# Tuxliri/RL_rocket

Hardware: AMD Instinct MI355X
Metric: env-steps/sec (6DOF, N=65536 per GPU) (higher is better)
Workload: dtype fp32

## Files before the change

### rl_rocket_amd/batch.py

```python
import ctypes

import numpy as np

from . import _lib
from .params import lower, make_config


def _ptr(t):
    return ctypes.c_void_p(t.data_ptr()) if t is not None else None


def _host_view(addr, shape, dtype):
    nbytes = int(np.prod(shape)) * np.dtype(dtype).itemsize
    return np.frombuffer((ctypes.c_char * nbytes).from_address(addr), dtype=dtype).reshape(shape)


class HostArray:

    def __init__(self, shape, dtype):
        self._lib = _lib.load()
        nbytes = max(1, int(np.prod(shape)) * np.dtype(dtype).itemsize)
        p = ctypes.c_void_p()
        _lib.check(self._lib.rr_host_alloc(ctypes.byref(p), nbytes), "rr_host_alloc")
        self.ptr = p
# ... 195 lines not shown
    def checkpoint(self):
        t = self.torch
        st, v0, _ = self.get_state()
        cw = t.empty((self.num_envs,), dtype=t.int32, device=self.device)
        ret = t.empty((self.num_envs,), dtype=t.float32, device=self.device)
        _lib.check(self.lib.rr_get_aux(self._h, _ptr(cw), _ptr(ret), self._stream()), "rr_get_aux")
        return {"state": st, "v0": v0, "counter": cw, "ep_return": ret}

    def restore(self, ck):
        self.set_state(ck["state"], v0=ck["v0"], elapsed=ck["counter"])
        cw, ret = ck["counter"].contiguous(), ck["ep_return"].contiguous()
        self._keep_aux = (cw, ret)
        _lib.check(self.lib.rr_set_aux(self._h, _ptr(cw), _ptr(ret), self._stream()), "rr_set_aux")

    def set_state64(self, state_soa, v0=None, elapsed=None):
        t = self.torch
        st = t.as_tensor(state_soa, device=self.device, dtype=t.float64).reshape(self.state_dim, self.num_envs)
        st = st.contiguous()
        v = None if v0 is None else t.as_tensor(v0, device=self.device, dtype=t.float32).reshape(-1).contiguous()
        el = None if elapsed is None else t.as_tensor(elapsed, device=self.device, dtype=t.int32).reshape(-1).contiguous()
        self._keep = (st, v, el)
        _lib.check(self.lib.rr_set_state64(self._h, _ptr(st), _ptr(v), _ptr(el), self._stream()), "rr_set_state64")

    def get_state64(self):
        t = self.torch
        st = t.empty((self.state_dim, self.num_envs), dtype=t.float64, device=self.device)
        v = t.empty((self.num_envs,), dtype=t.float32, device=self.device)
        el = t.empty((self.num_envs,), dtype=t.int32, device=self.device)
        _lib.check(self.lib.rr_get_state64(self._h, _ptr(st), _ptr(v), _ptr(el), self._stream()), "rr_get_state64")
        return st, v, el

    def fetch_done(self, capacity=None):
        cap = self.num_envs if capacity is None else min(int(capacity), self.num_envs)
        rows = min(cap, max(4096, len(self._fetch[0].array) if getattr(self, "_fetch", None) else 0))
        while True:
            if getattr(self, "_fetch", None) is None or len(self._fetch[0].array) < rows:
                self._free_fetch()
                ns = self.state_dim
                self._fetch = (HostArray((rows,), np.int32), HostArray((rows, ns), np.float32),
                               HostArray((rows,), np.float32), HostArray((rows,), np.int32))
            bufs = self._fetch
            c = self.lib.rr_fetch_done(self._h, min(cap, rows), *(b.ptr for b in bufs), self._stream())
            _lib.check(c, "rr_fetch_done")
            if int(c) <= rows or rows >= cap:
                break
            rows = min(cap, 1 << (int(c) - 1).bit_length())
        m = min(int(c), cap)
        return tuple(b.array[:m].copy() for b in bufs)

    def _free_fetch(self):
        for b in getattr(self, "_fetch", None) or ():
            b.free()
        self._fetch = None

    def copy_terminal(self, out=None):
        t = self.torch
        if out is None:
            out = (t.zeros((self.num_envs, self.state_dim), dtype=t.float32, device=self.device),
                   t.zeros((self.num_envs,), dtype=t.float32, device=self.device),
                   t.zeros((self.num_envs,), dtype=t.int32, device=self.device))
        tobs, ret, ln = out
        _lib.check(self.lib.rr_copy_terminal(self._h, _ptr(tobs), _ptr(ret), _ptr(ln), self._stream()),
                   "rr_copy_terminal")
        return tobs, ret, ln

    def close(self):
        if getattr(self, "_h", None) is not None and self._h.value:
            self.torch.cuda.synchronize(self.device)
            self.lib.rr_destroy(self._h)
            self._h = ctypes.c_void_p()
        self._free_fetch()

    def __del__(self):
        try:
            self.close()
        except Exception:
            pass
```

### rl_rocket_amd/build.py

```python
import os
import shutil
import subprocess
import sys

HERE = os.path.dirname(os.path.abspath(__file__))
ROOT = os.path.dirname(HERE)
SRC = os.path.join(HERE, "csrc", "rocket_hip.hip")
SRC_EXACT = os.path.join(HERE, "csrc", "rocket_exact.hip")
EXACT_FLAGS = ["-mllvm", "-amdgpu-schedule-metric-bias=100"]
SRC_COLLECT = os.path.join(HERE, "csrc", "rocket_collect.hip")
COLLECT_FLAGS = ["-mllvm", "-amdgpu-mfma-vgpr-form"]
SRC_EVAL_TRACE = os.path.join(HERE, "csrc", "eval_trace", "rocket_eval_trace.hip")
SRC_EVAL_EXACT = os.path.join(HERE, "csrc", "eval_exact", "rocket_eval_exact.hip")
EVAL_EXACT_FLAGS = EXACT_FLAGS + COLLECT_FLAGS
SRC_COLLECT_STATS = os.path.join(HERE, "csrc", "collect_stats", "rocket_collect_stats.hip")
INC_COLLECT_STATS = os.path.join(HERE, "csrc", "collect_stats", "rocket_collect_stats.inc")
SRC_PPO_OPTS = os.path.join(HERE, "csrc", "ppo_opts", "rocket_ppo_opts.hip")
SRC_BC = os.path.join(HERE, "csrc", "bc", "rocket_bc.hip")
SRC_DISCRETE = os.path.join(HERE, "csrc", "discrete", "rocket_discrete.hip")
HEADER = os.path.join(ROOT, "include", "rocket_hip.h")
OUT = os.path.join(HERE, "librocket_hip.so")
BENCH_SRC = os.path.join(ROOT, "tools", "bench_timed.hip")
BENCH_OUT = os.path.join(ROOT, "tools", "libbench_timed.so")
ARCH = os.environ.get("RR_OFFLOAD_ARCH", "gfx950")


def hipcc():
    for c in (os.environ.get("HIPCC"), shutil.which("hipcc"), "/opt/rocm/bin/hipcc"):
        if c and os.path.exists(c):
            return c
    raise RuntimeError("hipcc not found")


def command(resource_usage=False, out=OUT, defines=(), extra=(), src=SRC, compile_only=False, preload=4):
    cmd = [hipcc(), "--offload-arch=%s" % ARCH, "-O3", "-fno-slp-vectorize", "-ffp-contract=on", "-std=c++17",
           "-fPIC", "-c" if compile_only else "-shared"] + \
        (["-mllvm", "-amdgpu-kernarg-preload-count=%d" % preload] if preload else []) + \
        ["-I", os.path.join(ROOT, "include"), "-I", os.path.join(HERE, "csrc")] + list(extra) + \
        ["-D%s" % d for d in defines] + ["-o", out, src]
    if resource_usage:
        cmd.insert(1, "-Rpass-analysis=kernel-resource-usage")
    return cmd


def sources():
    csrc = os.path.join(HERE, "csrc")
    return sorted([os.path.join(csrc, f) for f in os.listdir(csrc) if os.path.isfile(os.path.join(csrc, f))]
                  + [SRC_EVAL_TRACE, SRC_EVAL_EXACT, SRC_COLLECT_STATS, INC_COLLECT_STATS, SRC_PPO_OPTS, SRC_BC, SRC_DISCRETE,
                     HEADER])


def source_hash():
    import hashlib

    h = hashlib.sha256()
    for path in sources():
        with open(path, "rb") as f:
            h.update(f.read())
    for cmd in commands():
        h.update(" ".join(cmd[1:]).replace(ROOT, "").encode())
    return h.hexdigest()[:16]


def commands(resource_usage=False, out=OUT, defines=(), extra=(), preload=4):
    o_main, o_exact, o_coll, o_trace = out + ".main.o", out + ".exact.o", out + ".collect.o", out + ".evaltrace.o"
    o_evx = out + ".evalexact.o"
    c1 = command(resource_usage, o_main, defines, extra, SRC, compile_only=True, preload=preload)
    c2 = command(resource_usage, o_exact, defines, list(extra) + EXACT_FLAGS, SRC_EXACT, compile_only=True,
                 preload=preload)
    c3 = command(resource_usage, o_coll, defines, list(extra) + COLLECT_FLAGS, SRC_COLLECT, compile_only=True,
                 preload=preload)
    c4 = command(resource_usage, o_trace, defines, list(extra) + COLLECT_FLAGS, SRC_EVAL_TRACE, compile_only=True,
                 preload=preload)
    c5 = command(resource_usage, o_evx, defines, list(extra) + EVAL_EXACT_FLAGS, SRC_EVAL_EXACT, compile_only=True,
                 preload=preload)
    objs = [o_main, o_exact, o_coll, o_trace, o_evx]
    c6 = command(resource_usage, out, defines, list(extra) + COLLECT_FLAGS + objs + [SRC_PPO_OPTS, SRC_BC, SRC_DISCRETE],
                 SRC_COLLECT_STATS,
                 preload=preload)
    return [c1, c2, c3, c4, c5, c6]


def build_lib(out=OUT, defines=(), extra=(), resource_usage=False, verbose=True, preload=4):
    cmds = commands(resource_usage, out, defines, extra, preload=preload)
    if verbose:
        for c in cmds:
            print("[rl_rocket_amd.build]", " ".join(c), flush=True)
    procs = [subprocess.Popen(c, cwd=ROOT) for c in cmds[:-1]]
    rcs = [p.wait() for p in procs]
    for c, rc in zip(cmds, rcs):
        if rc:
            raise subprocess.CalledProcessError(rc, c)
    subprocess.check_call(cmds[-1], cwd=ROOT)
    for c in cmds[:-1]:
        os.remove(c[c.index("-o") + 1])
    return out


def _llvm(tool):
    for d in (os.environ.get("ROCM_PATH", "/opt/rocm") + "/lib/llvm/bin", "/opt/rocm/llvm/bin"):
        if os.path.exists(os.path.join(d, tool)):
            return os.path.join(d, tool)
    found = shutil.which(tool)
    if not found:
        raise RuntimeError("%s not found" % tool)
    return found


def _elf_symbols(blob):
    import struct
# ... 85 lines not shown
```

### rl_rocket_amd/csrc/rocket_hip.hip

```cpp


#include <algorithm>
#include <cmath>
#include <cstdlib>
#include <cstring>
#include <new>
#include <string>
#include <vector>

#include "rocket_device.h"
#define RR_POL_PREFETCH_A 0
#include "rocket_policy.inc"
#include "rocket_rollout.inc"
#include "rocket_eval.inc"
#include "rocket_ppo.inc"

namespace {

__device__ __forceinline__ void entry_barrier()
{
    __builtin_amdgcn_fence(__ATOMIC_RELEASE, "workgroup", "local");
    __builtin_amdgcn_s_barrier();
    __builtin_amdgcn_fence(__ATOMIC_ACQUIRE, "workgroup", "local");
}

template <int MODEL, int INTEG, bool ASOA, bool HELP, int WPB, bool ROWS>
__global__ __launch_bounds__(HELP ? 2 * WPB * kWave : WPB * kWave) __attribute__((amdgpu_waves_per_eu(4))) void step_kernel(
    float* __restrict__ state, const float* __restrict__ action, uint32_t n_envs, uint32_t mode, const KParams P,
    const Bufs B, const StepIO io)
{
    constexpr int NS = Dims<MODEL>::NS, NA = Dims<MODEL>::NA, NT = Dims<MODEL>::NT, EV = Dims<MODEL>::EV;
    constexpr int OW = ROWS ? NS + 2 : NS;
    __shared__ __attribute__((aligned(16))) float lds[WPB][kWave * OW];
    constexpr int kCandRow = (NS + 1 + 3) / 4 * 4;
    __shared__ __attribute__((aligned(16))) float cand[HELP ? WPB : 1][HELP ? kWave * kCandRow : 1];
    __shared__ uint32_t cflag[WPB];
    const uint32_t lane = threadIdx.x & (kWave - 1);
    const uint32_t wv = __builtin_amdgcn_readfirstlane(threadIdx.x / kWave);
    const uint32_t n = n_envs;
    RR_STAMPS_BEGIN(4);
    RR_SUB_BEGIN(3);
    if constexpr (HELP) {
        if (wv >= (uint32_t)WPB) {
            const KParams& P = *B.kp;
            const uint32_t k = wv - WPB;
            const uint32_t base = (blockIdx.x * WPB + k) * kWave;
            const uint32_t ih = min(base + lane, n - 1);
            const uint32_t cwh = (base < n && (mode & kModeCounter)) ? at(B.counter, ih) : 0u;
// ... 142 lines not shown
    const int64_t i = (int64_t)blockIdx.x * kBlock + threadIdx.x;
    if (i >= B.n) return;
    const int64_t n = B.n;
    float s[NS], v0;
    if (mask == nullptr || mask[i]) {
        const uint32_t ep = (B.counter[i] >> P.ep_shift) + 1u;
        ResetStream key = reset_stream(B.kp->seed_w, P.id_off + i, B.counter[i]);
        sample_ic<MODEL>(P, key, s, v0);
#pragma unroll
        for (int j = 0; j < NS; ++j) B.state[(int64_t)j * n + i] = s[j];
        if (state64) {
#pragma unroll
            for (int j = 0; j < NS; ++j) state64[(int64_t)j * n + i] = (double)s[j];
        }
        B.v0[i] = v0;
        B.counter[i] = ep << P.ep_shift;
        B.ep_ret[i] = 0.0f;
    } else {
#pragma unroll
        for (int j = 0; j < NS; ++j) s[j] = B.state[(int64_t)j * n + i];
    }
    if (obs) {
#pragma unroll
        for (int j = 0; j < NS; ++j) obs[i * NS + j] = s[j] * P.inv_norm[j];
    }
}

__global__ __launch_bounds__(kBlock) void clear_elapsed_kernel(uint32_t* counter, int64_t n, uint32_t el_mask)
{
    const int64_t i = (int64_t)blockIdx.x * kBlock + threadIdx.x;
    if (i < n) counter[i] &= ~el_mask;
}

__global__ __launch_bounds__(kBlock) void gather_done_kernel(const int32_t* idx, int64_t count, int ns,
                                                             const float* term_obs, const float* term_ret,
                                                             const int32_t* term_len, const uint8_t* trunc,
                                                             float* g_obs, float* g_ret, int32_t* g_len,
                                                             uint8_t* g_trunc)
{
    const int64_t k = (int64_t)blockIdx.x * kBlock + threadIdx.x;
    if (k >= count) return;
    const int64_t i = idx[k];
    for (int j = 0; j < ns; ++j) g_obs[k * ns + j] = term_obs[i * ns + j];
    g_ret[k] = term_ret[i];
    g_len[k] = term_len[i];
    if (trunc) g_trunc[k] = trunc[i];
}

__global__ __launch_bounds__(kBlock) void copy_done_rows_kernel(const uint64_t* done_bits, int64_t n, int ns,
                                                                const float* term_obs, const float* term_ret,
                                                                const int32_t* term_len, float* d_obs, float* d_ret,
                                                                int32_t* d_len)
{
    const int64_t i = (int64_t)blockIdx.x * kBlock + threadIdx.x;
    if (i >= n || !((done_bits[i / kWave] >> (i % kWave)) & 1ull)) return;
    if (d_obs)
        for (int j = 0; j < ns; ++j) d_obs[i * ns + j] = term_obs[i * ns + j];
    if (d_ret) d_ret[i] = term_ret[i];
    if (d_len) d_len[i] = term_len[i];
}

__global__ __launch_bounds__(kBlock) void gae_kernel(int64_t T, int64_t n, const float* __restrict__ rewards,
                                                     const float* __restrict__ values,
                                                     const float* __restrict__ starts,
                                                     const float* __restrict__ last_value,
                                                     const float* __restrict__ last_done, double gamma, double lam,
                                                     float* __restrict__ adv, float* __restrict__ ret)
{
    const int64_t e = (int64_t)blockIdx.x * kBlock + threadIdx.x;
    if (e >= n) return;
    pol::gae_env(T, n, e, rewards, values, starts, last_value[e], last_done[e], gamma, lam, adv, ret);
}

__global__ __launch_bounds__(kBlock) void widen_kernel(const float* src, double* dst, int64_t count)
{
    const int64_t k = (int64_t)blockIdx.x * kBlock + threadIdx.x;
    if (k < count) dst[k] = (double)src[k];
}

__global__ __launch_bounds__(kBlock) void narrow_kernel(const double* src, float* dst, int64_t count)
{
    const int64_t k = (int64_t)blockIdx.x * kBlock + threadIdx.x;
    if (k < count) dst[k] = (float)src[k];
}

}

constexpr int kNoUnit = (int)hipErrorInvalidDeviceFunction;
extern "C" {
__attribute__((weak)) int rrx_launch_exact(const void*, const void*) { return kNoUnit; }
__attribute__((weak)) int rrx_launch_eval_exact(const void*, const void*) { return kNoUnit; }
__attribute__((weak)) int rrc_launch_collect(const void*, const void*) { return kNoUnit; }
__attribute__((weak)) int rrc_launch_eval(const void*, const void*) { return kNoUnit; }
__attribute__((weak)) int rrc_launch_eval_trace(const void*, const void*, const void*) { return kNoUnit; }
__attribute__((weak)) int rrc_launch_collect_stats(const void*, const void*, const void*) { return kNoUnit; }
__attribute__((weak)) int rrc_launch_learner(const void*, void*) { return kNoUnit; }
__attribute__((weak)) int rrc_launch_learner_opts(const void*, void*) { return kNoUnit; }
__attribute__((weak)) int rrc_launch_bc(const void*, void*) { return kNoUnit; }
__attribute__((weak)) int rrc_launch_discrete(const void*, void*) { return kNoUnit; }
}

namespace {

thread_local std::string g_err;

int fail(int code, const std::string& msg)
{
    g_err = msg;
    return code;
}

int hip_fail(hipError_t e, const char* what)
{
    return fail(RR_EHIP, std::string(what) + ": " + hipGetErrorString(e));
}

float ceil_f(double d)
{
    float f = (float)d;
    if ((double)f < d) f = std::nextafter(f, INFINITY);
    return f;
}
float floor_f(double d)
{
    float f = (float)d;
    if ((double)f > d) f = std::nextafter(f, -INFINITY);
    return f;
}

uint64_t splitmix64(uint64_t x)
{
    uint64_t z = x + 0x9E3779B97F4A7C15ull;
// ... 126 lines not shown
                if (M > pi) x.land_always |= 1u << ax;
                else x.land_c[ax] = std::cos(M);
            }
        }
    }
    return x;
}

}

struct rr_env {
    int device;
    rr_params p;
    KParams kp;
    XParams xp;
    int ns, na, nt;
    int64_t n, id_off;
    uint64_t steps;
    int64_t help_max_n;
    int64_t exact_lean_min_n;
    int64_t whole_line_min_n;
    float* state;
    float* v0;
    uint32_t* counter;
    float* ep_ret;
    uint64_t* done_bits;
    float* term_obs;
    float* term_ret;
    int32_t* term_len;
    double* state64;
    bool host_state;
    KParams* d_kp;
    XParams* d_xp;
    int32_t* g_idx;
    float* g_obs;
    float* g_ret;
    int32_t* g_len;
    uint8_t* g_trunc;
    static constexpr int kSeedStreams = 8;
    void* streams[kSeedStreams];
    int n_streams;
    bool streams_overflow;
    hipEvent_t seed_ev;
};

namespace {

inline void note_stream(rr_env* e, void* stream)
{
    if (e->n_streams > 0 && e->streams[e->n_streams - 1] == stream) return;
    for (int k = 0; k < e->n_streams; ++k)
        if (e->streams[k] == stream) {
            for (int j = k; j + 1 < e->n_streams; ++j) e->streams[j] = e->streams[j + 1];
            e->streams[e->n_streams - 1] = stream;
            return;
        }
    if (e->n_streams < rr_env::kSeedStreams) e->streams[e->n_streams++] = stream;
    else e->streams_overflow = true;
}

Bufs bufs_of(const rr_env* e)
{
    Bufs b;
    b.state = e->state;
    b.v0 = e->v0;
    b.counter = e->counter;
    b.ep_ret = e->ep_ret;
    b.done_bits = e->done_bits;
    b.term_obs = e->term_obs;
    b.term_ret = e->term_ret;
    b.term_len = e->term_len;
// ... 57 lines not shown
    if (p->flags & ~kKnownFlags)
        return fail(RR_EINVAL, "rr_create: unknown flag bits");
    rr_env* e = new (std::nothrow) rr_env();
    if (!e) return fail(RR_ENOMEM, "rr_create: host allocation failed");
    e->device = device;
    e->p = *p;
    e->kp = make_kparams(*p);
    e->xp = make_xparams(*p);
    e->ns = p->model == RR_MODEL_6DOF ? 14 : 7;
    e->na = p->model == RR_MODEL_6DOF ? 3 : 2;
    e->nt = p->model == RR_MODEL_6DOF ? 5 : 6;
    e->n = n;
    e->id_off = env_id_offset;
    DeviceGuard g(device);
    {
        const char* hv = std::getenv("RR_HELP_MAX_N");
        e->help_max_n = hv ? std::strtoll(hv, nullptr, 10) : kHelpMaxN;
        int cus = 0;
        if (hipDeviceGetAttribute(&cus, hipDeviceAttributeMultiprocessorCount, device) != hipSuccess || cus <= 0)
            cus = (int)kExactLeanCUs;
        const char* lv = std::getenv("RR_EXACT_LEAN_MIN_N");
        e->exact_lean_min_n = lv ? std::strtoll(lv, nullptr, 10) : (int64_t)cus * 4 * kWave;
        const char* wv = std::getenv("RR_WHOLE_LINE_MIN_N");
        e->whole_line_min_n = wv ? std::strtoll(wv, nullptr, 10) : kWholeLineMinN;
    }
    struct A {
        void** ptr;
        size_t bytes;
    } allocs[] = {
        {(void**)&e->state, sizeof(float) * (e->ns + 3) * n},
        {(void**)&e->done_bits, sizeof(uint64_t) * n_words(n)},
        {(void**)&e->term_obs, sizeof(float) * e->ns * n},
        {(void**)&e->term_ret, sizeof(float) * n},        {(void**)&e->term_len, sizeof(int32_t) * n},
        {(void**)&e->g_idx, sizeof(int32_t) * n},         {(void**)&e->g_obs, sizeof(float) * e->ns * n},
        {(void**)&e->g_ret, sizeof(float) * n},           {(void**)&e->g_len, sizeof(int32_t) * n},
        {(void**)&e->g_trunc, sizeof(uint8_t) * n},
    };
    const bool exact = p->integrator == RR_INT_DOPRI5;
    e->host_state = (p->flags & RR_FLAG_HOST_STATE) != 0;
    for (auto& a : allocs) {
        if (e->host_state && a.ptr == (void**)&e->state) {
            hipError_t err = hipHostMalloc(a.ptr, a.bytes, hipHostMallocCoherent | hipHostMallocMapped);
            if (err != hipSuccess) {
                *a.ptr = nullptr;
                rr_destroy(e);
                return hip_fail(err, "rr_create: hipHostMalloc (host state)");
            }
            std::memset(*a.ptr, 0, a.bytes);
            continue;
        }
        hipError_t err = hipMalloc(a.ptr, a.bytes);
        if (err != hipSuccess) {
            rr_destroy(e);
            return hip_fail(err, "rr_create: hipMalloc");
        }
        err = hipMemset(*a.ptr, 0, a.bytes);
        if (err != hipSuccess) {
            rr_destroy(e);
            return hip_fail(err, "rr_create: hipMemset");
        }
    }
    if (exact) {
        const size_t bytes = sizeof(double) * e->ns * n;
        hipError_t err = hipMalloc((void**)&e->state64, bytes);
        if (err == hipSuccess) err = hipMemset(e->state64, 0, bytes);
        if (err != hipSuccess) {
            rr_destroy(e);
            return hip_fail(err, "rr_create: hipMalloc (fp64 state)");
        }
    }
    e->v0 = e->state + (size_t)e->ns * n;
    e->counter = reinterpret_cast<uint32_t*>(e->state + (size_t)(e->ns + 1) * n);
    e->ep_ret = e->state + (size_t)(e->ns + 2) * n;
    e->kp.id_off = env_id_offset;
    {
        hipError_t err = hipMalloc((void**)&e->d_kp, sizeof(KParams));
        if (err == hipSuccess) err = hipEventCreateWithFlags(&e->seed_ev, hipEventDisableTiming);
        if (err == hipSuccess) err = hipMalloc((void**)&e->d_xp, sizeof(XParams));
        if (err == hipSuccess) err = hipMemcpy(e->d_xp, &e->xp, sizeof(XParams), hipMemcpyHostToDevice);
        if (err != hipSuccess) {
            rr_destroy(e);
            return hip_fail(err, "rr_create: hipMalloc (params)");
        }
    }
    int rc = rr_seed(e, 42, nullptr);
    if (rc == RR_OK) {
        hipError_t err = hipDeviceSynchronize();
        if (err != hipSuccess) rc = hip_fail(err, "rr_create: sync");
    }
    if (rc != RR_OK) {
        rr_destroy(e);
        return rc;
    }
    *out = e;
    return RR_OK;
}

int rr_destroy(rr_env* e)
{
    if (!e) return RR_OK;
    DeviceGuard g(e->device);
    if (e->host_state && e->state) {
        (void)hipHostFree(e->state);
        e->state = nullptr;
    }
    if (e->seed_ev) (void)hipEventDestroy(e->seed_ev);
    void* ptrs[] = {e->state, e->state64, e->d_kp, e->d_xp, e->done_bits,
                    e->term_obs, e->term_ret, e->term_len, e->g_idx, e->g_obs,  e->g_ret, e->g_len,
                    e->g_trunc};
    for (void* q : ptrs)
        if (q) (void)hipFree(q);
    delete e;
    return RR_OK;
}

int64_t rr_num_envs(const rr_env* e) { return e ? e->n : -1; }
int rr_state_dim(const rr_env* e) { return e ? e->ns : -1; }
int rr_action_dim(const rr_env* e) { return e ? e->na : -1; }

int rr_seed(rr_env* e, uint64_t seed, void* stream)
{
    if (!e) return fail(RR_EINVAL, "rr_seed: null handle");
    DeviceGuard g(e->device);
    hipStream_t s = (hipStream_t)stream;
    hipStreamCaptureStatus cs = hipStreamCaptureStatusNone;
    hipError_t err = hipStreamIsCapturing(s, &cs);
    if (err != hipSuccess) return hip_fail(err, "rr_seed: hipStreamIsCapturing");
    if (cs != hipStreamCaptureStatusNone)
        return fail(RR_EINVAL, "rr_seed: the stream is being captured into a graph (seed before capturing: "
                               "replays read the key current when they run)");
    bool sync_device = e->streams_overflow;
    for (int k = 0; k < e->n_streams && !sync_device; ++k) {
        hipStream_t o = (hipStream_t)e->streams[k];
        if (o == s) continue;
        hipStreamCaptureStatus ocs = hipStreamCaptureStatusNone;
        if (hipStreamIsCapturing(o, &ocs) != hipSuccess) {
            (void)hipGetLastError();
            sync_device = true;
            break;
        }
        if (ocs != hipStreamCaptureStatusNone) continue;
        err = hipEventRecord(e->seed_ev, o);
// ... 241 lines not shown
    out->v0 = e->v0;
    out->elapsed = (int32_t*)e->counter;
    out->ep_return = e->ep_ret;
    out->done_bits = e->done_bits;
    out->terminal_obs = e->term_obs;
    out->terminal_return = e->term_ret;
    out->terminal_len = e->term_len;
    return RR_OK;
}

int rr_host_alloc(void** out, int64_t bytes)
{
    if (!out || bytes <= 0) return fail(RR_EINVAL, "rr_host_alloc: null pointer or bytes <= 0");
    *out = nullptr;
    const hipError_t err = hipHostMalloc(out, (size_t)bytes, hipHostMallocCoherent | hipHostMallocMapped);
    if (err != hipSuccess) {
        *out = nullptr;
        return hip_fail(err, "rr_host_alloc");
    }
    std::memset(*out, 0, (size_t)bytes);
    return RR_OK;
}

int rr_host_free(void* p)
{
    if (!p) return RR_OK;
    const hipError_t err = hipHostFree(p);
    return err == hipSuccess ? RR_OK : hip_fail(err, "rr_host_free");
}

}

namespace {
int64_t fetch_rows(rr_env* e, const std::vector<int32_t>& hidx, int64_t capacity, const float* src_obs,
                   const float* src_ret, const int32_t* src_len, const uint8_t* src_trunc, int32_t* idx,
                   float* term_obs, float* term_return, int32_t* term_len, uint8_t* trunc_out, hipStream_t s,
                   const char* what)
{
    const int64_t count = (int64_t)hidx.size();
    const int64_t m = std::min<int64_t>(count, capacity);
    if (m == 0) return count;
    if (idx) std::memcpy(idx, hidx.data(), sizeof(int32_t) * m);
    if (term_obs || term_return || term_len || trunc_out) {
        hipError_t err = hipMemcpyAsync(e->g_idx, hidx.data(), sizeof(int32_t) * m, hipMemcpyHostToDevice, s);
        if (err != hipSuccess) return hip_fail(err, what);
        hipLaunchKernelGGL(gather_done_kernel, dim3(grid_of(m)), dim3(kBlock), 0, s, e->g_idx, m, e->ns, src_obs,
                           src_ret, src_len, trunc_out ? src_trunc : nullptr, e->g_obs, e->g_ret, e->g_len, e->g_trunc);
        err = hipGetLastError();
        if (err == hipSuccess && term_obs)
            err = hipMemcpyAsync(term_obs, e->g_obs, sizeof(float) * e->ns * m, hipMemcpyDefault, s);
        if (err == hipSuccess && term_return)
            err = hipMemcpyAsync(term_return, e->g_ret, sizeof(float) * m, hipMemcpyDefault, s);
        if (err == hipSuccess && term_len)
            err = hipMemcpyAsync(term_len, e->g_len, sizeof(int32_t) * m, hipMemcpyDefault, s);
        if (err == hipSuccess && trunc_out)
            err = hipMemcpyAsync(trunc_out, e->g_trunc, sizeof(uint8_t) * m, hipMemcpyDefault, s);
        if (err == hipSuccess) err = hipStreamSynchronize(s);
        if (err != hipSuccess) return hip_fail(err, what);
    }
    return count;
}
}

extern "C" {

int64_t rr_fetch_done(rr_env* e, int64_t capacity, int32_t* idx, float* term_obs, float* term_return,
                      int32_t* term_len, void* stream)
{
    if (!e) return fail(RR_EINVAL, "rr_fetch_done: null handle");
    if (capacity < 0) return fail(RR_EINVAL, "rr_fetch_done: negative capacity");
    if (e->steps == 0) return 0;
    hipStream_t s = (hipStream_t)stream;
    const int64_t nw = n_words(e->n);
    std::vector<uint64_t> bits(nw);
    hipError_t err = hipMemcpyAsync(bits.data(), e->done_bits, sizeof(uint64_t) * nw, hipMemcpyDeviceToHost, s);
    if (err == hipSuccess) err = hipStreamSynchronize(s);
    if (err != hipSuccess) return hip_fail(err, "rr_fetch_done: done bits");
    std::vector<int32_t> hidx;
    for (int64_t w = 0; w < nw; ++w) {
        uint64_t m = bits[w];
        while (m) {
            const int b = __builtin_ctzll(m);
            hidx.push_back((int32_t)(w * kWave + b));
            m &= m - 1;
        }
    }
    return fetch_rows(e, hidx, capacity, e->term_obs, e->term_ret, e->term_len, nullptr, idx, term_obs, term_return,
                      term_len, nullptr, s, "rr_fetch_done: gather");
}

int64_t rr_gather_rows(rr_env* e, const uint8_t* done, const float* term_obs_src, const float* term_return_src,
                       const int32_t* term_len_src, const uint8_t* truncated_src, int64_t capacity, int32_t* idx,
                       float* term_obs, float* term_return, int32_t* term_len, uint8_t* truncated, void* stream)
{
    if (!e || !done) return fail(RR_EINVAL, "rr_gather_rows: null handle or done flags");
    if (capacity < 0) return fail(RR_EINVAL, "rr_gather_rows: negative capacity");
    if ((term_obs && !term_obs_src) || (term_return && !term_return_src) || (term_len && !term_len_src) ||
        (truncated && !truncated_src))
        return fail(RR_EINVAL, "rr_gather_rows: an output without its source");
    hipStream_t s = (hipStream_t)stream;
    const int64_t n = e->n;
    std::vector<uint64_t> flags((n + 7) / 8, 0);
    hipError_t err = hipMemcpyAsync(flags.data(), done, (size_t)n, hipMemcpyDefault, s);
    if (err == hipSuccess) err = hipStreamSynchronize(s);
    if (err != hipSuccess) return hip_fail(err, "rr_gather_rows: done flags");
    std::vector<int32_t> hidx;
    const uint8_t* f8 = reinterpret_cast<const uint8_t*>(flags.data());
    for (int64_t w = 0; w < (int64_t)flags.size(); ++w) {
        if (!flags[w]) continue;
        for (int64_t i = 8 * w; i < std::min<int64_t>(8 * w + 8, n); ++i)
            if (f8[i]) hidx.push_back((int32_t)i);
    }
    return fetch_rows(e, hidx, capacity, term_obs_src, term_return_src, term_len_src, truncated_src, idx, term_obs,
                      term_return, term_len, truncated, s, "rr_gather_rows: gather");
}

int rr_copy_terminal(rr_env* e, float* term_obs, float* term_return, int32_t* term_len, void* stream)
{
    if (!e) return fail(RR_EINVAL, "rr_copy_terminal: null handle");
    if (!term_obs && !term_return && !term_len) return RR_OK;
    if (e->steps == 0) return RR_OK;
    hipLaunchKernelGGL(copy_done_rows_kernel, dim3(grid_of(e->n)), dim3(kBlock), 0, (hipStream_t)stream,
                       e->done_bits, e->n, e->ns, e->term_obs, e->term_ret, e->term_len, term_obs, term_return,
                       term_len);
    hipError_t err = hipGetLastError();
    return err == hipSuccess ? RR_OK : hip_fail(err, "rr_copy_terminal");
}


}

static int prec_of(int precision)
{
    return precision == RR_POLICY_FP32 ? 0 : precision == RR_POLICY_BF16 ? 1 : precision == RR_POLICY_FP16X3 ? 2 : -1;
}

template <class F>
static bool pol_dispatch(int obs_dim, int act_dim, int precision, F&& f)
{
    const int prec = prec_of(precision);
    if (prec < 0) return false;
    if (obs_dim == 14 && act_dim == 3) dispatch_prec(prec, [&](auto p) { f(tag<14>{}, tag<3>{}, p); });
    else if (obs_dim == 7 && act_dim == 2) dispatch_prec(prec, [&](auto p) { f(tag<7>{}, tag<2>{}, p); });
    else return false;
    return true;
}

// ... 871 lines not shown
```

### rl_rocket_amd/vec_env.py

```python
import itertools
import time
from collections.abc import Sequence

import numpy as np

from . import _lib
from .batch import RocketBatch
from .gym_compat import Box
from .params import MAX_EPISODE_STEPS, parse_model

try:
    from stable_baselines3.common.vec_env.base_vec_env import VecEnv as _VecEnvBase
except Exception:
    _VecEnvBase = object


class _DoneRows:

    def __init__(self, idx, tobs, ret, ln, trunc, max_episode_steps, monitor, stamp):
        self.idx = np.asarray(idx)
        self._pos = None
        self.tobs, self.ret, self.ln, self.trunc = tobs, ret, ln, trunc
        self.max_steps = max_episode_steps
        self.monitor = monitor
# ... 232 lines not shown
        t.cuda.current_stream(self.batch.device).synchronize()
        o, r, d, tr = (v.numpy() for v in views)
        return o, r, d.view(np.bool_), tr

    def _now(self):
        return round(time.time() - self._t_start, 6)

    def _done_rows(self, idx, tobs, ret, ln, trunc_k, now):
        if self.monitor:
            self.episode_returns.extend(ret.tolist())
            self.episode_lengths.extend(ln.tolist())
            self.episode_times.extend([now] * len(idx))
        return _DoneRows(idx, tobs, ret, ln, trunc_k, self.max_episode_steps, self.monitor, now)

    def _init_device_sets(self):
        t = self.batch.torch
        n, ns, dev = self.num_envs, self.batch.state_dim, self.batch.device
        self._sets = []
        for _ in range(2):
            self._sets.append({
                "out": self.batch.alloc_outputs(),
                "term": (t.empty((n, ns), dtype=t.float32, device=dev), t.empty((n,), dtype=t.float32, device=dev),
                         t.empty((n,), dtype=t.int32, device=dev)),
                "terms": None if self.batch.terms is None else t.empty_like(self.batch.terms),
                "infos": None,
            })
        self._slot = 0
        self._pending = []
        self._gbuf = {}

    def _gather_done(self, done, trunc, term, stamp):
        import ctypes

        from .batch import HostArray

        n, ns = self.num_envs, self.batch.state_dim
        g = self._gbuf
        if g.get("rows") is None:
            g["rows"] = (HostArray((n,), np.int32), HostArray((n, ns), np.float32), HostArray((n,), np.float32),
                         HostArray((n,), np.int32), HostArray((n,), np.uint8))
        h = g["rows"]
        P = ctypes.c_void_p
        tobs, ret, ln = term
        c = self.batch.lib.rr_gather_rows(
            self.batch._h, P(done.data_ptr()), P(tobs.data_ptr()), P(ret.data_ptr()), P(ln.data_ptr()),
            P(trunc.data_ptr()), n, *(b.ptr for b in h), self.batch._stream())
        _lib.check(c, "rr_gather_rows")
        m = int(c)
        if not m:
            return None
        idx, tobs_h, ret_h, ln_h, tr_h = (b.array[:m].copy() for b in h)
        return self._done_rows(idx, tobs_h, ret_h, ln_h, tr_h, stamp)

    def _flush_all(self):
        while self._pending:
            self._pending[0]._build()

    def _step_device(self):
        tm = self.timing
        if tm is not None:
            t0 = time.perf_counter()
        self._slot ^= 1
        st = self._sets[self._slot]
        old = st["infos"]
        if old is not None:
            if self.monitor:
                old._build()
            else:
                old._drop()
        if tm is not None:
            t1 = time.perf_counter()
        obs, rew, done, trunc = self.batch.step(self._actions, out=st["out"])
        self.batch.copy_terminal(out=st["term"])
        if st["terms"] is not None:
            st["terms"].copy_(self.batch.terms)
        infos = _DeviceInfos(self, st, self._now())
        st["infos"] = infos
        self._pending.append(infos)
        if tm is not None:
            t2 = time.perf_counter()
            for k, v in (("infos", t1 - t0), ("launch", t2 - t1)):
                tm[k] = tm.get(k, 0.0) + v
        return obs, rew, done.bool(), infos

    def close(self):
        if self.device_outputs and getattr(self, "_pending", None):
            self._flush_all()
        self.batch.close()
        for b in (getattr(self, "_gbuf", None) or {}).get("rows") or ():
            b.free()

    def seed(self, seed=None):
        if seed is None:
            seed = int(np.random.randint(0, 2 ** 31 - 1))
        self.batch.seed(seed)
        return [seed + i for i in range(self.num_envs)]

    def _indices(self, indices):
        if indices is None:
            return range(self.num_envs)
        if isinstance(indices, int):
            return [indices]
        return indices

    def get_attr(self, attr_name, indices=None):
        value = getattr(self, attr_name, None)
        if value is None:
            value = getattr(self.batch.cfg, attr_name, None)
        if value is None and attr_name in self.batch.cfg.kwargs:
            value = self.batch.cfg.kwargs[attr_name]
        if value is None and attr_name == "reward_coefficients":
            value = self.batch.cfg.kwargs["reward_coeff"]
        return [value for _ in self._indices(indices)]

    def set_attr(self, attr_name, value, indices=None):
        raise AttributeError("RocketVecEnv envs share one device-resident config; %r cannot be set per env"
                             % attr_name)

    def env_method(self, method_name, *method_args, indices=None, **method_kwargs):
        raise AttributeError("RocketVecEnv has no per-env python objects (method %r)" % method_name)

    def env_is_wrapped(self, wrapper_class, indices=None):
        name = getattr(wrapper_class, "__name__", "")
# ... 31 lines not shown
```

Measured before the change: 17.30 billion.

## Compact done rows on device into mapped host memory instead of host scan

Replaces the host-side done-bit download, CPU index scan, index upload, gather kernel, and multiple device-to-host copies with on-device count and compaction kernels. These write indices and terminal rows straight into a coherent mapped pinned block, which the host then memcpy's into plain numpy buffers. The aim is to cut round trips and host scanning in the done-fetch path. In exchange it adds two kernel launches per fetch, a regrow-and-retry loop, and slower writes to coherent host memory.

```diff
diff --git a/rl_rocket_amd/batch.py b/rl_rocket_amd/batch.py
--- a/rl_rocket_amd/batch.py
+++ b/rl_rocket_amd/batch.py
@@ -251,26 +251,20 @@
 
     def fetch_done(self, capacity=None):
         cap = self.num_envs if capacity is None else min(int(capacity), self.num_envs)
-        rows = min(cap, max(4096, len(self._fetch[0].array) if getattr(self, "_fetch", None) else 0))
+        rows = min(cap, max(4096, len(self._fetch[0]) if getattr(self, "_fetch", None) else 0))
         while True:
-            if getattr(self, "_fetch", None) is None or len(self._fetch[0].array) < rows:
-                self._free_fetch()
+            if getattr(self, "_fetch", None) is None or len(self._fetch[0]) < rows:
                 ns = self.state_dim
-                self._fetch = (HostArray((rows,), np.int32), HostArray((rows, ns), np.float32),
-                               HostArray((rows,), np.float32), HostArray((rows,), np.int32))
+                self._fetch = (np.empty((rows,), np.int32), np.empty((rows, ns), np.float32),
+                               np.empty((rows,), np.float32), np.empty((rows,), np.int32))
             bufs = self._fetch
-            c = self.lib.rr_fetch_done(self._h, min(cap, rows), *(b.ptr for b in bufs), self._stream())
+            c = self.lib.rr_fetch_done(self._h, min(cap, rows), *(b.ctypes.data for b in bufs), self._stream())
             _lib.check(c, "rr_fetch_done")
             if int(c) <= rows or rows >= cap:
                 break
             rows = min(cap, 1 << (int(c) - 1).bit_length())
         m = min(int(c), cap)
-        return tuple(b.array[:m].copy() for b in bufs)
-
-    def _free_fetch(self):
-        for b in getattr(self, "_fetch", None) or ():
-            b.free()
-        self._fetch = None
+        return tuple(b[:m].copy() for b in bufs)
 
     def copy_terminal(self, out=None):
         t = self.torch
@@ -288,7 +282,6 @@
             self.torch.cuda.synchronize(self.device)
             self.lib.rr_destroy(self._h)
             self._h = ctypes.c_void_p()
-        self._free_fetch()
 
     def __del__(self):
         try:
diff --git a/rl_rocket_amd/build.py b/rl_rocket_amd/build.py
--- a/rl_rocket_amd/build.py
+++ b/rl_rocket_amd/build.py
@@ -18,6 +18,8 @@
 SRC_PPO_OPTS = os.path.join(HERE, "csrc", "ppo_opts", "rocket_ppo_opts.hip")
 SRC_BC = os.path.join(HERE, "csrc", "bc", "rocket_bc.hip")
 SRC_DISCRETE = os.path.join(HERE, "csrc", "discrete", "rocket_discrete.hip")
+SRC_DONE_FETCH = os.path.join(HERE, "csrc", "done_fetch", "rocket_done_fetch.hip")
+INC_DONE_FETCH = os.path.join(HERE, "csrc", "done_fetch", "rocket_done_fetch.h")
 HEADER = os.path.join(ROOT, "include", "rocket_hip.h")
 OUT = os.path.join(HERE, "librocket_hip.so")
 BENCH_SRC = os.path.join(ROOT, "tools", "bench_timed.hip")
@@ -47,7 +49,7 @@
     csrc = os.path.join(HERE, "csrc")
     return sorted([os.path.join(csrc, f) for f in os.listdir(csrc) if os.path.isfile(os.path.join(csrc, f))]
                   + [SRC_EVAL_TRACE, SRC_EVAL_EXACT, SRC_COLLECT_STATS, INC_COLLECT_STATS, SRC_PPO_OPTS, SRC_BC, SRC_DISCRETE,
-                     HEADER])
+                     SRC_DONE_FETCH, INC_DONE_FETCH, HEADER])
 
 
 def source_hash():
@@ -75,7 +77,7 @@
     c5 = command(resource_usage, o_evx, defines, list(extra) + EVAL_EXACT_FLAGS, SRC_EVAL_EXACT, compile_only=True,
                  preload=preload)
     objs = [o_main, o_exact, o_coll, o_trace, o_evx]
-    c6 = command(resource_usage, out, defines, list(extra) + COLLECT_FLAGS + objs + [SRC_PPO_OPTS, SRC_BC, SRC_DISCRETE],
+    c6 = command(resource_usage, out, defines, list(extra) + COLLECT_FLAGS + objs + [SRC_PPO_OPTS, SRC_BC, SRC_DISCRETE, SRC_DONE_FETCH],
                  SRC_COLLECT_STATS,
                  preload=preload)
     return [c1, c2, c3, c4, c5, c6]
diff --git a/rl_rocket_amd/csrc/done_fetch/rocket_done_fetch.h b/rl_rocket_amd/csrc/done_fetch/rocket_done_fetch.h
--- /dev/null
+++ b/rl_rocket_amd/csrc/done_fetch/rocket_done_fetch.h
@@ -0,0 +1,44 @@
+#pragma once
+#include <cstdint>
+#include <type_traits>
+
+namespace done_fetch {
+
+constexpr int kThreads = 1024;
+constexpr int64_t kEnvsPerBlock = (int64_t)kThreads * 64;
+constexpr int64_t kStartRows = 1024;
+
+struct State {
+    void* block;
+    int64_t rows;
+    uint32_t* totals;
+};
+
+struct Fetch {
+    const uint64_t* bits;
+    const uint8_t* flags;
+    int64_t n;
+    int ns;
+    int device;
+    const float* src_obs;
+    const float* src_ret;
+    const int32_t* src_len;
+    const uint8_t* src_trunc;
+    int64_t capacity;
+    int32_t* idx;
+    float* obs;
+    float* ret;
+    int32_t* len;
+    uint8_t* trunc;
+    void* stream;
+};
+static_assert(std::is_trivially_copyable_v<State> && std::is_trivially_copyable_v<Fetch>, "cross TUs by pointer");
+
+}
+
+extern "C" {
+__attribute__((visibility("hidden"))) int rrd_done_state_init(done_fetch::State* st, int64_t n);
+__attribute__((visibility("hidden"))) void rrd_done_state_free(done_fetch::State* st);
+__attribute__((visibility("hidden"))) int rrd_done_fetch(done_fetch::State* st, const done_fetch::Fetch* f,
+                                                         int64_t* count);
+}
diff --git a/rl_rocket_amd/csrc/done_fetch/rocket_done_fetch.hip b/rl_rocket_amd/csrc/done_fetch/rocket_done_fetch.hip
--- /dev/null
+++ b/rl_rocket_amd/csrc/done_fetch/rocket_done_fetch.hip
@@ -0,0 +1,294 @@
+#include <hip/hip_runtime.h>
+
+#include <algorithm>
+#include <cstring>
+
+#include "done_fetch/rocket_done_fetch.h"
+
+namespace {
+
+using done_fetch::kEnvsPerBlock;
+using done_fetch::kThreads;
+constexpr int kSlices = 32;
+constexpr int kSliceWords = kThreads / kSlices;
+constexpr int kWave = 64;
+constexpr int kWaves = kThreads / kWave;
+
+struct Sections {
+    int64_t* count;
+    int32_t* idx;
+    float* obs;
+    float* ret;
+    int32_t* len;
+    uint8_t* trunc;
+};
+
+constexpr size_t kHead = 64;
+
+size_t block_bytes(int64_t rows, int ns) { return kHead + (size_t)rows * (4 + 4 * (size_t)ns + 4 + 4 + 1); }
+
+__host__ __device__ inline Sections sections(void* block, int64_t rows, int ns)
+{
+    Sections s;
+    char* p = static_cast<char*>(block);
+    s.count = reinterpret_cast<int64_t*>(p);
+    p += kHead;
+    s.idx = reinterpret_cast<int32_t*>(p);
+    p += 4 * rows;
+    s.obs = reinterpret_cast<float*>(p);
+    p += 4 * rows * ns;
+    s.ret = reinterpret_cast<float*>(p);
+    p += 4 * rows;
+    s.len = reinterpret_cast<int32_t*>(p);
+    p += 4 * rows;
+    s.trunc = reinterpret_cast<uint8_t*>(p);
+    return s;
+}
+
+__device__ __forceinline__ uint32_t nonzero_bytes(uint64_t x)
+{
+    x |= x >> 4;
+    x |= x >> 2;
+    x |= x >> 1;
+    x &= 0x0101010101010101ull;
+    return (uint32_t)((x * 0x0102040810204080ull) >> 56);
+}
+
+__device__ __forceinline__ uint64_t done_mask(const uint64_t* __restrict__ bits, const uint8_t* __restrict__ flags,
+                                              int64_t n, int64_t w, bool wide)
+{
+    const int64_t e0 = w * kWave;
+    if (e0 >= n) return 0;
+    const int64_t live = n - e0;
+    uint64_t m = 0;
+    if (bits) {
+        m = bits[w];
+    } else if (wide && live >= kWave) {
+        const uint4* q = reinterpret_cast<const uint4*>(flags + e0);
+#pragma unroll
+        for (int k = 0; k < 4; ++k) {
+            const uint4 v = q[k];
+            const uint64_t lo = (uint64_t)v.x | ((uint64_t)v.y << 32), hi = (uint64_t)v.z | ((uint64_t)v.w << 32);
+            m |= (uint64_t)(nonzero_bytes(lo) | (nonzero_bytes(hi) << 8)) << (16 * k);
+        }
+    } else {
+        const int cnt = live < kWave ? (int)live : kWave;
+        for (int k = 0; k < cnt; ++k) m |= (uint64_t)(flags[e0 + k] != 0) << k;
+    }
+    if (live < kWave) m &= (1ull << live) - 1ull;
+    return m;
+}
+
+__device__ __forceinline__ void block_scan(uint32_t a, uint32_t b, uint32_t* red, uint32_t& excl, uint32_t& sum_a,
+                                           uint32_t& sum_b)
+{
+    const int lane = threadIdx.x % kWave, wave = threadIdx.x / kWave;
+    uint32_t inc = a, tb = b;
+#pragma unroll
+    for (int d = 1; d < kWave; d *= 2) {
+        const uint32_t up = __shfl_up(inc, d, kWave);
+        if (lane >= d) inc += up;
+        tb += __shfl_xor(tb, d, kWave);
+    }
+    if (lane == kWave - 1) red[wave] = inc;
+    if (lane == 0) red[kWaves + wave] = tb;
+    __syncthreads();
+    uint32_t before = 0;
+    sum_a = 0;
+    sum_b = 0;
+#pragma unroll
+    for (int k = 0; k < kWaves; ++k) {
+        const uint32_t t = red[k];
+        if (k < wave) before += t;
+        sum_a += t;
+        sum_b += red[kWaves + k];
+    }
+    excl = before + inc - a;
+    __syncthreads();
+}
+
+__global__ __launch_bounds__(kThreads) void done_count_kernel(const uint64_t* __restrict__ bits,
+                                                              const uint8_t* __restrict__ flags, int64_t n, int wide,
+                                                              uint32_t* __restrict__ totals)
+{
+    __shared__ uint32_t red[2 * kWaves];
+    const int64_t w = (int64_t)blockIdx.x * kThreads + threadIdx.x;
+    const uint32_t c = (uint32_t)__popcll(done_mask(bits, flags, n, w, wide != 0));
+    uint32_t excl, sum, unused;
+    block_scan(c, 0u, red, excl, sum, unused);
+    if (threadIdx.x == 0) totals[blockIdx.x] = sum;
+}
+
+struct Sources {
+    const float* obs;
+    const float* ret;
+    const int32_t* len;
+    const uint8_t* trunc;
+};
+
+template <class PIECE>
+__global__ __launch_bounds__(kThreads) void done_compact_kernel(const uint64_t* __restrict__ bits,
+                                                                const uint8_t* __restrict__ flags, int64_t n, int ns,
+                                                                int wide, const uint32_t* __restrict__ totals,
+                                                                Sources src, void* block, int64_t block_rows, int64_t rows,
+                                                                int want_idx)
+{
+    __shared__ uint32_t red[2 * kWaves];
+    __shared__ uint32_t lim[2];
+    __shared__ int32_t sidx[kSliceWords * kWave];
+    const unsigned seg = blockIdx.x / kSlices, slice = blockIdx.x % kSlices, nseg = gridDim.x / kSlices;
+    const int64_t w = (int64_t)seg * kThreads + threadIdx.x;
+    uint64_t m = done_mask(bits, flags, n, w, wide != 0);
+    const uint32_t c = (uint32_t)__popcll(m);
+    uint32_t excl, mine, unused;
+    block_scan(c, 0u, red, excl, mine, unused);
+    int64_t base = 0, total = mine;
+    if (totals) {
+        uint32_t pa = 0, pb = 0;
+        for (unsigned k = threadIdx.x; k < nseg; k += kThreads) {
+            const uint32_t t = totals[k];
+            pa += k < seg ? t : 0u;
+            pb += t;
+        }
+        uint32_t e2, before, all;
+        block_scan(pa, pb, red, e2, before, all);
+        base = before;
+        total = all;
+    }
+    const Sections out = sections(block, block_rows, ns);
+    if (blockIdx.x == 0 && threadIdx.x == 0) *out.count = total;
+    const bool in_slice = threadIdx.x / kSliceWords == slice;
+    if (threadIdx.x == slice * kSliceWords) lim[0] = excl;
+    if (threadIdx.x == slice * kSliceWords + kSliceWords - 1) lim[1] = excl + c;
+    __syncthreads();
+    const int64_t first = base + lim[0];
+    const int64_t end = base + lim[1] < rows ? base + lim[1] : rows;
+    if (first >= end) return;
+    if (in_slice)
+        for (int64_t p = base + excl; m && p < end; ++p) {
+            sidx[p - first] = (int32_t)(w * kWave + __builtin_ctzll(m));
+            m &= m - 1;
+        }
+    __syncthreads();
+    const int64_t cnt = end - first;
+    for (int64_t k = threadIdx.x; k < cnt; k += kThreads) {
+        const int64_t p = first + k, i = sidx[k];
+        if (want_idx) out.idx[p] = (int32_t)i;
+        if (src.ret) out.ret[p] = src.ret[i];
+        if (src.len) out.len[p] = src.len[i];
+        if (src.trunc) out.trunc[p] = src.trunc[i];
+    }
+    if (src.obs) {
+        const PIECE* __restrict__ so = reinterpret_cast<const PIECE*>(src.obs);
+        PIECE* __restrict__ dobs = reinterpret_cast<PIECE*>(out.obs);
+        const uint32_t ppr = (uint32_t)ns / (uint32_t)(sizeof(PIECE) / sizeof(float)), pieces = (uint32_t)cnt * ppr;
+        for (uint32_t q = threadIdx.x; q < pieces; q += kThreads) {
+            const uint32_t k = q / ppr, j = q - k * ppr;
+            const int64_t i = sidx[k];
+            dobs[(first + k) * ppr + j] = so[i * ppr + j];
+        }
+    }
+}
+
+int64_t round_rows(int64_t r) { return (r + 15) / 16 * 16; }
+
+hipError_t alloc_block(done_fetch::State* st, int64_t rows, int ns)
+{
+    void* p = nullptr;
+    const size_t bytes = block_bytes(rows, ns);
+    const hipError_t err = hipHostMalloc(&p, bytes, hipHostMallocCoherent | hipHostMallocMapped);
+    if (err != hipSuccess) return err;
+    std::memset(p, 0, bytes);
+    if (st->block) (void)hipHostFree(st->block);
+    st->block = p;
+    st->rows = rows;
+    return hipSuccess;
+}
+
+struct DeviceGuard {
+    int prev = -1;
+    explicit DeviceGuard(int dev)
+    {
+        if (hipGetDevice(&prev) != hipSuccess) prev = -1;
+        if (prev != dev) (void)hipSetDevice(dev);
+    }
+    ~DeviceGuard()
+    {
+        if (prev >= 0) (void)hipSetDevice(prev);
+    }
+};
+
+}
+
+extern "C" int rrd_done_state_init(done_fetch::State* st, int64_t n)
+{
+    *st = done_fetch::State{};
+    const size_t bytes = sizeof(uint32_t) * (size_t)((n + kEnvsPerBlock - 1) / kEnvsPerBlock);
+    hipError_t err = hipMalloc((void**)&st->totals, bytes);
+    if (err == hipSuccess) err = hipMemset(st->totals, 0, bytes);
+    return (int)err;
+}
+
+extern "C" void rrd_done_state_free(done_fetch::State* st)
+{
+    if (st->block) (void)hipHostFree(st->block);
+    if (st->totals) (void)hipFree(st->totals);
+    *st = done_fetch::State{};
+}
+
+extern "C" int rrd_done_fetch(done_fetch::State* st, const done_fetch::Fetch* fp, int64_t* count)
+{
+    const done_fetch::Fetch f = *fp;
+    hipStream_t s = (hipStream_t)f.stream;
+    const int64_t nblocks = (f.n + kEnvsPerBlock - 1) / kEnvsPerBlock;
+    const int64_t want = std::min(f.capacity, f.n);
+    const int wide = f.flags && (reinterpret_cast<uintptr_t>(f.flags) % 16 == 0);
+    const Sources src = {f.obs ? f.src_obs : nullptr, f.ret ? f.src_ret : nullptr, f.len ? f.src_len : nullptr,
+                         f.trunc ? f.src_trunc : nullptr};
+    const bool pairs = f.ns % 2 == 0 && reinterpret_cast<uintptr_t>(src.obs) % 8 == 0;
+    if (!st->block) {
+        DeviceGuard g(f.device);
+        const hipError_t err = alloc_block(st, round_rows(std::min<int64_t>(f.n, done_fetch::kStartRows)), f.ns);
+        if (err != hipSuccess) return (int)err;
+    }
+    for (;;) {
+        const int64_t rows = std::min(want, st->rows);
+        const uint32_t* totals = nullptr;
+        if (nblocks > 1) {
+            hipLaunchKernelGGL(done_count_kernel, dim3((unsigned)nblocks), dim3(kThreads), 0, s, f.bits, f.flags, f.n,
+                               wide, st->totals);
+            totals = st->totals;
+        }
+        if (pairs)
+            hipLaunchKernelGGL(done_compact_kernel<float2>, dim3((unsigned)nblocks * kSlices), dim3(kThreads), 0, s, f.bits,
+                               f.flags, f.n, f.ns, wide, totals, src, st->block, st->rows, rows,
+                               f.idx ? 1 : 0);
+        else
+            hipLaunchKernelGGL(done_compact_kernel<float>, dim3((unsigned)nblocks * kSlices), dim3(kThreads), 0, s, f.bits,
+                               f.flags, f.n, f.ns, wide, totals, src, st->block, st->rows, rows,
+                               f.idx ? 1 : 0);
+        hipError_t err = hipGetLastError();
+        if (err == hipSuccess) err = hipStreamSynchronize(s);
+        if (err != hipSuccess) return (int)err;
+        const Sections sec = sections(st->block, st->rows, f.ns);
+        const int64_t c = *sec.count;
+        const int64_t m = std::min(c, want);
+        if (m > rows) {
+            int64_t r = st->rows;
+            while (r < m) r *= 2;
+            DeviceGuard g(f.device);
+            err = alloc_block(st, round_rows(std::min(r, f.n)), f.ns);
+            if (err != hipSuccess) return (int)err;
+            continue;
+        }
+        if (m > 0) {
+            if (f.idx) std::memcpy(f.idx, sec.idx, sizeof(int32_t) * m);
+            if (f.obs) std::memcpy(f.obs, sec.obs, sizeof(float) * f.ns * m);
+            if (f.ret) std::memcpy(f.ret, sec.ret, sizeof(float) * m);
+            if (f.len) std::memcpy(f.len, sec.len, sizeof(int32_t) * m);
+            if (f.trunc) std::memcpy(f.trunc, sec.trunc, sizeof(uint8_t) * m);
+        }
+        *count = c;
+        return (int)hipSuccess;
+    }
+}
diff --git a/rl_rocket_amd/csrc/rocket_hip.hip b/rl_rocket_amd/csrc/rocket_hip.hip
--- a/rl_rocket_amd/csrc/rocket_hip.hip
+++ b/rl_rocket_amd/csrc/rocket_hip.hip
@@ -14,6 +14,7 @@
 #include "rocket_rollout.inc"
 #include "rocket_eval.inc"
 #include "rocket_ppo.inc"
+#include "done_fetch/rocket_done_fetch.h"
 
 namespace {
 
@@ -222,21 +223,6 @@
     if (i < n) counter[i] &= ~el_mask;
 }
 
-__global__ __launch_bounds__(kBlock) void gather_done_kernel(const int32_t* idx, int64_t count, int ns,
-                                                             const float* term_obs, const float* term_ret,
-                                                             const int32_t* term_len, const uint8_t* trunc,
-                                                             float* g_obs, float* g_ret, int32_t* g_len,
-                                                             uint8_t* g_trunc)
-{
-    const int64_t k = (int64_t)blockIdx.x * kBlock + threadIdx.x;
-    if (k >= count) return;
-    const int64_t i = idx[k];
-    for (int j = 0; j < ns; ++j) g_obs[k * ns + j] = term_obs[i * ns + j];
-    g_ret[k] = term_ret[i];
-    g_len[k] = term_len[i];
-    if (trunc) g_trunc[k] = trunc[i];
-}
-
 __global__ __launch_bounds__(kBlock) void copy_done_rows_kernel(const uint64_t* done_bits, int64_t n, int ns,
                                                                 const float* term_obs, const float* term_ret,
                                                                 const int32_t* term_len, float* d_obs, float* d_ret,
@@ -288,6 +274,13 @@
 __attribute__((weak)) int rrc_launch_learner_opts(const void*, void*) { return kNoUnit; }
 __attribute__((weak)) int rrc_launch_bc(const void*, void*) { return kNoUnit; }
 __attribute__((weak)) int rrc_launch_discrete(const void*, void*) { return kNoUnit; }
+__attribute__((weak)) int rrd_done_state_init(done_fetch::State* st, int64_t)
+{
+    *st = done_fetch::State{};
+    return (int)hipSuccess;
+}
+__attribute__((weak)) void rrd_done_state_free(done_fetch::State*) {}
+__attribute__((weak)) int rrd_done_fetch(done_fetch::State*, const done_fetch::Fetch*, int64_t*) { return kNoUnit; }
 }
 
 namespace {
@@ -480,11 +473,7 @@
     bool host_state;
     KParams* d_kp;
     XParams* d_xp;
-    int32_t* g_idx;
-    float* g_obs;
-    float* g_ret;
-    int32_t* g_len;
-    uint8_t* g_trunc;
+    done_fetch::State fetch;
     static constexpr int kSeedStreams = 8;
     void* streams[kSeedStreams];
     int n_streams;
@@ -608,9 +597,6 @@
         {(void**)&e->done_bits, sizeof(uint64_t) * n_words(n)},
         {(void**)&e->term_obs, sizeof(float) * e->ns * n},
         {(void**)&e->term_ret, sizeof(float) * n},        {(void**)&e->term_len, sizeof(int32_t) * n},
-        {(void**)&e->g_idx, sizeof(int32_t) * n},         {(void**)&e->g_obs, sizeof(float) * e->ns * n},
-        {(void**)&e->g_ret, sizeof(float) * n},           {(void**)&e->g_len, sizeof(int32_t) * n},
-        {(void**)&e->g_trunc, sizeof(uint8_t) * n},
     };
     const bool exact = p->integrator == RR_INT_DOPRI5;
     e->host_state = (p->flags & RR_FLAG_HOST_STATE) != 0;
@@ -658,6 +644,11 @@
             rr_destroy(e);
             return hip_fail(err, "rr_create: hipMalloc (params)");
         }
+        err = (hipError_t)rrd_done_state_init(&e->fetch, n);
+        if (err != hipSuccess) {
+            rr_destroy(e);
+            return hip_fail(err, "rr_create: done-fetch scratch");
+        }
     }
     int rc = rr_seed(e, 42, nullptr);
     if (rc == RR_OK) {
@@ -681,9 +672,8 @@
         e->state = nullptr;
     }
     if (e->seed_ev) (void)hipEventDestroy(e->seed_ev);
-    void* ptrs[] = {e->state, e->state64, e->d_kp, e->d_xp, e->done_bits,
-                    e->term_obs, e->term_ret, e->term_len, e->g_idx, e->g_obs,  e->g_ret, e->g_len,
-                    e->g_trunc};
+    rrd_done_state_free(&e->fetch);
+    void* ptrs[] = {e->state, e->state64, e->d_kp, e->d_xp, e->done_bits, e->term_obs, e->term_ret, e->term_len};
     for (void* q : ptrs)
         if (q) (void)hipFree(q);
     delete e;
@@ -991,33 +981,31 @@
 }
 
 namespace {
-int64_t fetch_rows(rr_env* e, const std::vector<int32_t>& hidx, int64_t capacity, const float* src_obs,
+int64_t fetch_rows(rr_env* e, const uint64_t* bits, const uint8_t* flags, int64_t capacity, const float* src_obs,
                    const float* src_ret, const int32_t* src_len, const uint8_t* src_trunc, int32_t* idx,
-                   float* term_obs, float* term_return, int32_t* term_len, uint8_t* trunc_out, hipStream_t s,
+                   float* term_obs, float* term_return, int32_t* term_len, uint8_t* trunc_out, void* stream,
                    const char* what)
 {
-    const int64_t count = (int64_t)hidx.size();
-    const int64_t m = std::min<int64_t>(count, capacity);
-    if (m == 0) return count;
-    if (idx) std::memcpy(idx, hidx.data(), sizeof(int32_t) * m);
-    if (term_obs || term_return || term_len || trunc_out) {
-        hipError_t err = hipMemcpyAsync(e->g_idx, hidx.data(), sizeof(int32_t) * m, hipMemcpyHostToDevice, s);
-        if (err != hipSuccess) return hip_fail(err, what);
-        hipLaunchKernelGGL(gather_done_kernel, dim3(grid_of(m)), dim3(kBlock), 0, s, e->g_idx, m, e->ns, src_obs,
-                           src_ret, src_len, trunc_out ? src_trunc : nullptr, e->g_obs, e->g_ret, e->g_len, e->g_trunc);
-        err = hipGetLastError();
-        if (err == hipSuccess && term_obs)
-            err = hipMemcpyAsync(term_obs, e->g_obs, sizeof(float) * e->ns * m, hipMemcpyDefault, s);
-        if (err == hipSuccess && term_return)
-            err = hipMemcpyAsync(term_return, e->g_ret, sizeof(float) * m, hipMemcpyDefault, s);
-        if (err == hipSuccess && term_len)
-            err = hipMemcpyAsync(term_len, e->g_len, sizeof(int32_t) * m, hipMemcpyDefault, s);
-        if (err == hipSuccess && trunc_out)
-            err = hipMemcpyAsync(trunc_out, e->g_trunc, sizeof(uint8_t) * m, hipMemcpyDefault, s);
-        if (err == hipSuccess) err = hipStreamSynchronize(s);
-        if (err != hipSuccess) return hip_fail(err, what);
-    }
-    return count;
+    done_fetch::Fetch f{};
+    f.bits = bits;
+    f.flags = flags;
+    f.n = e->n;
+    f.ns = e->ns;
+    f.device = e->device;
+    f.src_obs = src_obs;
+    f.src_ret = src_ret;
+    f.src_len = src_len;
+    f.src_trunc = src_trunc;
+    f.capacity = capacity;
+    f.idx = idx;
+    f.obs = term_obs;
+    f.ret = term_return;
+    f.len = term_len;
+    f.trunc = trunc_out;
+    f.stream = stream;
+    int64_t count = 0;
+    const hipError_t err = (hipError_t)rrd_done_fetch(&e->fetch, &f, &count);
+    return err == hipSuccess ? count : hip_fail(err, what);
 }
 }
 
@@ -1029,23 +1017,8 @@
     if (!e) return fail(RR_EINVAL, "rr_fetch_done: null handle");
     if (capacity < 0) return fail(RR_EINVAL, "rr_fetch_done: negative capacity");
     if (e->steps == 0) return 0;
-    hipStream_t s = (hipStream_t)stream;
-    const int64_t nw = n_words(e->n);
-    std::vector<uint64_t> bits(nw);
-    hipError_t err = hipMemcpyAsync(bits.data(), e->done_bits, sizeof(uint64_t) * nw, hipMemcpyDeviceToHost, s);
-    if (err == hipSuccess) err = hipStreamSynchronize(s);
-    if (err != hipSuccess) return hip_fail(err, "rr_fetch_done: done bits");
-    std::vector<int32_t> hidx;
-    for (int64_t w = 0; w < nw; ++w) {
-        uint64_t m = bits[w];
-        while (m) {
-            const int b = __builtin_ctzll(m);
-            hidx.push_back((int32_t)(w * kWave + b));
-            m &= m - 1;
-        }
-    }
-    return fetch_rows(e, hidx, capacity, e->term_obs, e->term_ret, e->term_len, nullptr, idx, term_obs, term_return,
-                      term_len, nullptr, s, "rr_fetch_done: gather");
+    return fetch_rows(e, e->done_bits, nullptr, capacity, e->term_obs, e->term_ret, e->term_len, nullptr, idx,
+                      term_obs, term_return, term_len, nullptr, stream, "rr_fetch_done");
 }
 
 int64_t rr_gather_rows(rr_env* e, const uint8_t* done, const float* term_obs_src, const float* term_return_src,
@@ -1057,21 +1030,8 @@
     if ((term_obs && !term_obs_src) || (term_return && !term_return_src) || (term_len && !term_len_src) ||
         (truncated && !truncated_src))
         return fail(RR_EINVAL, "rr_gather_rows: an output without its source");
-    hipStream_t s = (hipStream_t)stream;
-    const int64_t n = e->n;
-    std::vector<uint64_t> flags((n + 7) / 8, 0);
-    hipError_t err = hipMemcpyAsync(flags.data(), done, (size_t)n, hipMemcpyDefault, s);
-    if (err == hipSuccess) err = hipStreamSynchronize(s);
-    if (err != hipSuccess) return hip_fail(err, "rr_gather_rows: done flags");
-    std::vector<int32_t> hidx;
-    const uint8_t* f8 = reinterpret_cast<const uint8_t*>(flags.data());
-    for (int64_t w = 0; w < (int64_t)flags.size(); ++w) {
-        if (!flags[w]) continue;
-        for (int64_t i = 8 * w; i < std::min<int64_t>(8 * w + 8, n); ++i)
-            if (f8[i]) hidx.push_back((int32_t)i);
-    }
-    return fetch_rows(e, hidx, capacity, term_obs_src, term_return_src, term_len_src, truncated_src, idx, term_obs,
-                      term_return, term_len, truncated, s, "rr_gather_rows: gather");
+    return fetch_rows(e, nullptr, done, capacity, term_obs_src, term_return_src, term_len_src, truncated_src, idx,
+                      term_obs, term_return, term_len, truncated, stream, "rr_gather_rows");
 }
 
 int rr_copy_terminal(rr_env* e, float* term_obs, float* term_return, int32_t* term_len, void* stream)
diff --git a/rl_rocket_amd/vec_env.py b/rl_rocket_amd/vec_env.py
--- a/rl_rocket_amd/vec_env.py
+++ b/rl_rocket_amd/vec_env.py
@@ -288,24 +288,22 @@
     def _gather_done(self, done, trunc, term, stamp):
         import ctypes
 
-        from .batch import HostArray
-
         n, ns = self.num_envs, self.batch.state_dim
         g = self._gbuf
         if g.get("rows") is None:
-            g["rows"] = (HostArray((n,), np.int32), HostArray((n, ns), np.float32), HostArray((n,), np.float32),
-                         HostArray((n,), np.int32), HostArray((n,), np.uint8))
+            g["rows"] = (np.empty((n,), np.int32), np.empty((n, ns), np.float32), np.empty((n,), np.float32),
+                         np.empty((n,), np.int32), np.empty((n,), np.uint8))
         h = g["rows"]
         P = ctypes.c_void_p
         tobs, ret, ln = term
         c = self.batch.lib.rr_gather_rows(
             self.batch._h, P(done.data_ptr()), P(tobs.data_ptr()), P(ret.data_ptr()), P(ln.data_ptr()),
-            P(trunc.data_ptr()), n, *(b.ptr for b in h), self.batch._stream())
+            P(trunc.data_ptr()), n, *(P(b.ctypes.data) for b in h), self.batch._stream())
         _lib.check(c, "rr_gather_rows")
         m = int(c)
         if not m:
             return None
-        idx, tobs_h, ret_h, ln_h, tr_h = (b.array[:m].copy() for b in h)
+        idx, tobs_h, ret_h, ln_h, tr_h = (b[:m].copy() for b in h)
         return self._done_rows(idx, tobs_h, ret_h, ln_h, tr_h, stamp)
 
     def _flush_all(self):
@@ -343,8 +341,6 @@
         if self.device_outputs and getattr(self, "_pending", None):
             self._flush_all()
         self.batch.close()
-        for b in (getattr(self, "_gbuf", None) or {}).get("rows") or ():
-            b.free()
 
     def seed(self, seed=None):
         if seed is None:
```

Measured after the change: 17.21 billion. About the same (-0.5%).
